# roahmlab/armour

Hardware: AMD Instinct MI355X
Metric: planning iters/s (eval_g+jac) Kinova 7-DOF, 100 timesteps × 20 obstacles (higher is better)
Workload: dtype f64

## Files before the change

### armour_amd/_lib.py

```python
import ctypes as C
import os

_HERE = os.path.dirname(os.path.abspath(__file__))
KEY128 = os.environ.get("ARMOUR_KEY128", "0") not in ("", "0")
LIB_PATH = os.environ.get("ARMOUR_HIP_LIB") or os.path.join(_HERE, "lib", "libarmour_hip_k128.so" if KEY128 else "libarmour_hip.so")

MAXJ = 9
MAXF = 8 if KEY128 else 7

OK, EINVAL, EDEVICE, ECAPACITY, ESTATE = 0, -1, -2, -3, -4
ROADMAP_KNN_MAX = 64
ROADMAP_KNN_MANY = 2048
TREE_NOT_FOUND, TREE_FOUND, TREE_START_BLOCKED, TREE_GOAL_BLOCKED, TREE_FULL = 0, 1, 2, 3, 4
TREE_MAX_NODES, TREE_MAX_ITERATIONS = 8192, 100000
SHORTCUT_OK, SHORTCUT_INVALID = 0, 1
SHORTCUT_MAX_POINTS, SHORTCUT_MAX_PASSES = 1024, 8


class ArmourRobot(C.Structure):
    _fields_ = [
        ("num_joints", C.c_int32), ("num_factors", C.c_int32),
        ("axes", C.c_int32 * MAXJ), ("continuous", C.c_int32 * MAXF),
        ("trans", C.c_double * ((MAXJ + 1) * 3)), ("rots", C.c_double * (MAXJ * 3)),
        ("mass", C.c_double * MAXJ), ("mass_uncertainty", C.c_double),
# ... 75 lines not shown
OPT_P1_TWO_PASS = 106
OPT_P1_STEP_PAIRS = 107
OPT_P1_STEP_QUEUE = 109
OPT_P1_STEP_TAIL_CROSS = 108
OPT_P1_STEP_TWO_CU = 123
OPT_P1_STEP_LEAN_BACK = 124
OPT_P1_TV_TAIL_CROSS = 121
OPT_P1_TV_MIN_GROUPS = 110
OPT_P1_TV_WAVES = 111
OPT_P1_TV_FREE = 112
OPT_P1_TV_SPLIT_FK = 113
OPT_P1_TV_DEDICATED = 114
OPT_P1_TV_HELP_SHIFT = 115
OPT_P1_TV_HELPERS = 116
OPT_P1_TV_HELP_MIN = 117
OPT_P1_TV_HELP_N = 118
OPT_P1_TV_AUX3 = 119
OPT_P1_FULL_PLANES = 120
OPT_P1_TV_ROW_WIDTH = 122
OPT_P2_EX = 130
OPT_STEPS_GRAPH_MIN = 131
OPT_PINNED_MODE = 132
OPT_CULL_ROWS = 133
OPT_SOLVE_SUB_TILES = 140
OPT_SOLVE_DEVICE = 141
OPT_SOLVE_CUT_TILES = 142
OPT_SOLVE_BLOCKS = 143
OPT_SOLVE_SUB_BATCH = 144
OPT_SOLVE_ROW_CAP = 145
OPT_SOLVE_HARD_CAP_S = 146
OPT_SOLVE_WAVES_PER_SIMD = 147
OPT_SOLVE_CULL = 148

EXPORTS = [
    "armour_robot_kinova_gen3_no_gripper", "armour_robot_kinova_gen3_gripper", "armour_robot_fetch", "armour_robot_fetch8", "armour_params_default", "armour_create", "armour_destroy",
    "armour_last_error", "armour_device_available", "armour_alloc_pinned", "armour_free_pinned", "armour_set_problems", "armour_set_problems_armtd", "armour_get_sizes",
    "armour_get_bounds", "armour_eval_f", "armour_eval_grad_f", "armour_eval_g_jac",
    "armour_eval_g_jac_device", "armour_eval_g_jac_device_steps", "armour_prepare_steps", "armour_eval_g_jac_device_multi", "armour_desired_trajectory", "armour_robust_controller", "armour_check_feasible", "armour_get_torque_radius",
    "armour_get_link_generators", "armour_get_link_centers", "armour_get_pz", "armour_get_table_sizes",
    "armour_solve_options_default", "armour_solve", "armour_debug_qp", "armour_debug_qp_box", "armour_debug_qp_elastic", "armour_debug_qp_device", "armour_debug_pz_op",
    "armour_get_hyperplanes", "armour_get_build_ms", "armour_get_build_info", "armour_p2_kernel_name", "armour_debug_load_tables",
    "armour_get_plane_skip", "armour_get_prune_margin", "armour_batch_get_prune_margin", "armour_set_option", "armour_get_option", "armour_controller_set_kernel", "armour_device_memory", "armour_abi_max_factors", "armour_eval_violations_device", "armour_eval_violations", "armour_get_row_relevance", "armour_get_solver_rows",
    "armour_batch_partition", "armour_batch_create", "armour_batch_destroy", "armour_batch_set_option", "armour_batch_set_problems",
    "armour_batch_get_sizes", "armour_batch_get_bounds", "armour_batch_eval_g_jac", "armour_batch_eval_violations", "armour_batch_solve",
    "armour_batch_get_build_ms", "armour_batch_get_build_info",
    "armour_roadmap_create", "armour_roadmap_destroy", "armour_roadmap_get_sizes", "armour_roadmap_check", "armour_roadmap_plan",
# ... 184 lines not shown
```

### armour_amd/csrc/api.hip

```cpp
#include <algorithm>
#include <cmath>
#include <cstdarg>
#include <chrono>
#include <cstring>
#include <mutex>
#include <new>

#include "../../include/armour_robot_fetch.h"
#include "../../include/armour_robot_kinova.h"
#include "bezier.h"
#include "cacc.h"
#include "common.h"
#include "solver_common.h"

static thread_local char g_err[512] = "";

void armour_set_error(const char* fmt, ...) {
    va_list ap;
    va_start(ap, fmt);
    vsnprintf(g_err, sizeof(g_err), fmt, ap);
    va_end(ap);
}

extern "C" const char* armour_last_error(void) { return g_err; }

extern "C" void armour_robot_kinova_gen3_no_gripper(ArmourRobot* robot) { armour_fill_kinova_gen3_no_gripper(robot); }
extern "C" void armour_robot_kinova_gen3_gripper(ArmourRobot* robot) { armour_fill_kinova_gen3_gripper(robot); }
extern "C" void armour_robot_fetch(ArmourRobot* robot) { armour_fill_fetch(robot); }
extern "C" int armour_robot_fetch8(ArmourRobot* robot) {
#if ARMOUR_MAX_FACTORS >= 8
    if (!robot) { armour_set_error("null argument"); return ARMOUR_EINVAL; }
    armour_fill_fetch8(robot);
    return ARMOUR_OK;
#else
    (void)robot;
// ... 78 lines not shown
    tb.row0 = h->row0; tb.mode = h->mode;
    tb.link_count = h->d_link_count; tb.link_center = h->d_link_center; tb.link_indep = h->d_link_indep;
    tb.link_keys = h->d_link_keys; tb.link_coeff = h->d_link_coeff;
    tb.tq_count = h->d_tq_count; tb.tq_center = h->d_tq_center; tb.tq_indep = h->d_tq_indep;
    tb.tq_keys = h->d_tq_keys; tb.tq_coeff = h->d_tq_coeff;
    tb.planes = h->d_planes; tb.planes_ll = h->d_planes_ll; tb.ll_shared = h->ll_shared;
    tb.ex_allowed = h->tune(ARMOUR_OPT_P2_EX);
    tb.obs_center = (h->d_from_center && (h->B >= 8 || !h->planes_have_d)) ? h->d_obs_center : nullptr;
    tb.plane_skip = h->d_plane_skip; tb.bez = h->d_bez;
    for (int i = 0; i < ARMOUR_MAX_FACTORS; i++) tb.k_range[i] = h->params.k_range[i];
    tb.duration = h->params.duration;
    return tb;
}

namespace {
struct TuningSpec { int option; double def, lo, hi; };
const TuningSpec kTuning[] = {
    {ARMOUR_OPT_P1_STEP_WAVES, 0, 0, 4}, {ARMOUR_OPT_P1_STEP_FREE, 1, 0, 1}, {ARMOUR_OPT_P1_STEP_SPLIT_FK, -1, -1, 1}, {ARMOUR_OPT_P1_STEP_AUX3, 1, 0, 1},
    {ARMOUR_OPT_P1_MAX_WAVES_PER_CU, 4, 1, 8}, {ARMOUR_OPT_P1_TWO_PASS, 1, 0, 1}, {ARMOUR_OPT_P1_STEP_PAIRS, 1, 0, 2}, {ARMOUR_OPT_P1_STEP_QUEUE, 1, 0, 3}, {ARMOUR_OPT_P1_STEP_TAIL_CROSS, 0, 0, 514}, {ARMOUR_OPT_P1_STEP_TWO_CU, 3, 0, 33}, {ARMOUR_OPT_P1_STEP_LEAN_BACK, 1, 0, 3}, {ARMOUR_OPT_P1_TV_TAIL_CROSS, 111, 0, 514} ,
    {ARMOUR_OPT_P1_TV_MIN_GROUPS, 31, 1, 1e6}, {ARMOUR_OPT_P1_TV_WAVES, 0, 0, 8}, {ARMOUR_OPT_P1_TV_FREE, 1, 0, 1}, {ARMOUR_OPT_P1_TV_SPLIT_FK, -1, -1, 1},
    {ARMOUR_OPT_P1_TV_DEDICATED, 1, 0, 1}, {ARMOUR_OPT_P1_TV_HELP_SHIFT, 0, 0, 3}, {ARMOUR_OPT_P1_TV_HELPERS, 1, 0, 31}, {ARMOUR_OPT_P1_TV_HELP_MIN, 192, 1, 1e6},
    {ARMOUR_OPT_P1_TV_HELP_N, 1, 0, 1}, {ARMOUR_OPT_P1_TV_AUX3, 1, 0, 1}, {ARMOUR_OPT_P1_TV_ROW_WIDTH, 0, 0, 64}, {ARMOUR_OPT_P1_FULL_PLANES, 0, 0, 1},
    {ARMOUR_OPT_P2_EX, 1, 0, 1}, {ARMOUR_OPT_STEPS_GRAPH_MIN, 2, 0, 1e6}, {ARMOUR_OPT_PINNED_MODE, 0, 0, 2}, {ARMOUR_OPT_CULL_ROWS, 0, 0, 1},
    {ARMOUR_OPT_SOLVE_SUB_TILES, 48, 1, 1e6}, {ARMOUR_OPT_SOLVE_DEVICE, 1, 0, 2}, {ARMOUR_OPT_SOLVE_CUT_TILES, 156, 1, 1e6}, {ARMOUR_OPT_SOLVE_BLOCKS, 0, 0, 1e6},
    {ARMOUR_OPT_SOLVE_SUB_BATCH, 0, 0, 1e6}, {ARMOUR_OPT_SOLVE_ROW_CAP, 0, 0, 1e7}, {ARMOUR_OPT_SOLVE_HARD_CAP_S, 0, 0, 1e6}, {ARMOUR_OPT_SOLVE_WAVES_PER_SIMD, 0, 0, 2}, {ARMOUR_OPT_SOLVE_CULL, -1, -1, 1},
};
const TuningSpec* tuning_spec(int option) {
    for (const TuningSpec& t : kTuning) if (t.option == option) return &t;
    return nullptr;
}
}
void armour_tuning_defaults(double* tuning) {
    for (int o = ARMOUR_OPT_FIRST_TUNING; o <= ARMOUR_OPT_LAST_TUNING; o++) tuning[o - ARMOUR_OPT_FIRST_TUNING] = 0.0;
    for (const TuningSpec& t : kTuning) tuning[t.option - ARMOUR_OPT_FIRST_TUNING] = t.def;
}
bool armour_trace_p1() { static const bool on = getenv("ARMOUR_P1_TRACE") != nullptr; return on; }
BuildStamps& armour_build_stamps() { static thread_local BuildStamps s; return s; }
void armour_build_stamp(const char* name) {
    if (!armour_trace_p1()) return;
    BuildStamps& s = armour_build_stamps();
    if (s.n < 12) { s.t[s.n] = std::chrono::duration<double, std::micro>(std::chrono::steady_clock::now().time_since_epoch()).count(); s.name[s.n] = name; s.n++; }
}
static void armour_build_stamps_print(const char* what) {
    if (!armour_trace_p1()) return;
    BuildStamps& s = armour_build_stamps();
    fprintf(stderr, "[%s, host side, us]", what);
// ... 51 lines not shown
    return ARMOUR_OK;
}

double* armour_handle_pinned(ArmourPlanner* h, int slot, size_t bytes) {
    if (h->solve_pin[slot] && h->solve_pin_bytes[slot] >= bytes) return static_cast<double*>(h->solve_pin[slot]);
    if (h->solve_pin[slot]) { armour_free_pinned(h->solve_pin[slot]); h->solve_pin[slot] = nullptr; h->solve_pin_bytes[slot] = 0; }
    void* p = nullptr;
    if (armour_alloc_pinned(bytes, &p) != ARMOUR_OK) return nullptr;
    h->solve_pin[slot] = p; h->solve_pin_bytes[slot] = bytes;
    return static_cast<double*>(p);
}

static void drop_step_graphs(ArmourPlanner* h) {
    for (auto& g : h->step_graphs) (void)hipGraphExecDestroy(g.exec);
    h->step_graphs.clear();
}

extern "C" void armour_destroy(ArmourPlanner* h) {
    if (!h) return;
    (void)hipSetDevice(h->device);
    if (h->stream) (void)hipStreamSynchronize(h->stream);
    drop_step_graphs(h);
    for (void* pin : h->solve_pin) armour_free_pinned(pin);
    armour_p1_free(h);
    if (h->stream) (void)hipStreamDestroy(h->stream);
    delete h;
}

static int begin_problem_set(ArmourPlanner* h, int B, int O, const double* q0, const double* qd0, const double* qdd0,
                             const double* q_des, int mode = ARMOUR_MODE_ARMOUR) {
    if (!h || !q0 || !qd0 || !qdd0 || !q_des) { armour_set_error("null argument"); return ARMOUR_EINVAL; }
    if (B < 1 || O < 0) { armour_set_error("bad batch/obstacle count (B=%d, O=%d)", B, O); return ARMOUR_EINVAL; }
    {
        const double* arrs[4] = {q0, qd0, qdd0, q_des};
        const size_t bn = (size_t)B * h->n;
        for (int a = 0; a < 4; a++)
            if (const size_t i = first_nonfinite(arrs[a], bn); i < bn) { armour_set_error("non-finite entry in the initial state / goal arrays (array %d, entry %zu)", a, i); return ARMOUR_EINVAL; }
    }
    HIPCHK(hipSetDevice(h->device));
    h->ready = false;
    h->rel.fresh = false; h->rel2.fresh = false;
    h->bounds_on_device = false; h->bounds_on_host = false;
    h->tables_from_host = false;
    h->stats_fresh = false;
    drop_step_graphs(h);
    int rc = ensure_capacity(h, B, O);
// ... 336 lines not shown
            }
    return enqueue_steps(h, d_k, steps, d_g, d_jac, st);
}

extern "C" int armour_eval_g_jac_device_multi(ArmourPlanner* h, const double* d_k, int32_t points, double* d_g, double* d_jac,
                                              void* stream) {
    NEED_READY(h);
    if (!d_k || points < 0) { armour_set_error("bad argument"); return ARMOUR_EINVAL; }
    if (points == 0) return ARMOUR_OK;
    const P2Tables tb = armour_make_tables(h);
    const long long bn = (long long)h->B * h->n, bm = (long long)h->B * h->m;
    return armour_p2_launch(tb, h->max_link, h->max_torque, h->h_plane_skip.data(), d_k, d_g, d_jac, stream ? (hipStream_t)stream : h->stream,
                            points, bn, bm, bm * h->n);
}

int armour_spin_on_stream(hipStream_t st) {
    for (;;) {
        const hipError_t q = hipStreamQuery(st);
        if (q == hipSuccess) return ARMOUR_OK;
        if (q != hipErrorNotReady) { armour_set_error("hipStreamQuery failed: %s", hipGetErrorString(q)); return ARMOUR_EDEVICE; }
    }
}

extern "C" int armour_eval_g_jac(ArmourPlanner* h, const double* k, double* g, double* jac) {
    NEED_READY(h);
    if (!k) { armour_set_error("k is null"); return ARMOUR_EINVAL; }
    HIPCHK(hipSetDevice(h->device));
    const size_t bn = (size_t)h->B * h->n, bm = (size_t)h->B * h->m;
    const P2Tables tb = armour_make_tables(h);
    const int pinned_mode = h->tune(ARMOUR_OPT_PINNED_MODE);
    const bool all_pinned = in_pinned(k, bn * sizeof(double)) && in_pinned(g, bm * sizeof(double)) && in_pinned(jac, bm * h->n * sizeof(double));
    if (all_pinned && pinned_mode == 1) {
        int rc = armour_p2_launch(tb, h->max_link, h->max_torque, h->h_plane_skip.data(), k, g, jac, h->stream);
        if (rc != ARMOUR_OK) return rc;
        return armour_spin_on_stream(h->stream);
    }
    const double* k_dev = h->d_k;
    if (all_pinned && pinned_mode == 2) k_dev = k;
    else HIPCHK(hipMemcpyAsync(h->d_k, k, bn * sizeof(double), hipMemcpyHostToDevice, h->stream));
    int rc = armour_p2_launch(tb, h->max_link, h->max_torque, h->h_plane_skip.data(), k_dev, g ? h->d_g : nullptr, jac ? h->d_jac : nullptr, h->stream);
    if (rc != ARMOUR_OK) return rc;
    if (g && jac && jac == g + bm) {
        HIPCHK(hipMemcpyAsync(g, h->d_g, bm * (1 + (size_t)h->n) * sizeof(double), hipMemcpyDeviceToHost, h->stream));
        return armour_spin_on_stream(h->stream);
    }
    if (g) HIPCHK(hipMemcpyAsync(g, h->d_g, bm * sizeof(double), hipMemcpyDeviceToHost, h->stream));
    if (jac) HIPCHK(hipMemcpyAsync(jac, h->d_jac, bm * h->n * sizeof(double), hipMemcpyDeviceToHost, h->stream));
    return armour_spin_on_stream(h->stream);
}

extern "C" int armour_check_feasible(ArmourPlanner* h, const double* g, int32_t* feasible) {
    NEED_READY(h);
    const slv::RowRule R = armour_row_rule(h);
    const slv::RowLimits L = armour_row_limits(h);
    for (int b = 0; b < h->B; b++) {
        const double* gb = g + (size_t)b * R.m;
        const double* tr = torque_radius_of(h, b);
        bool ok = true;
        for (int r = 0; r < R.m && ok; r++) {
            double l, u;
            slv::row_bounds(R, L, r, tr, &l, &u);
            ok = !slv::outside_slack(R, r, gb[r], l, u);
        }
        feasible[b] = ok ? 1 : 0;
// ... 90 lines not shown
    armour_set_error("armour_get_option: unknown option %d", option);
    return ARMOUR_EINVAL;
}

namespace {
struct ViolArgs {
    slv::RowRule rule;
    const double* g; const double* lo; const double* hi;
    ArmourViolation* out;
};
__global__ __launch_bounds__(256) void armour_violation_kernel(ViolArgs a) {
    __shared__ slv::ViolShared<1> sh;
    const int b = blockIdx.x, tid = threadIdx.x, m = a.rule.m;
    const double* g = a.g + (size_t)b * m;
    const double* lo = a.lo + (size_t)b * m;
    const double* hi = a.hi + (size_t)b * m;
    slv::ViolPartial p[1];
    for (int r = tid; r < m; r += 256) p[0].take(a.rule, r, g[r], lo[r], hi[r]);
    slv::ViolPartial::tree_reduce(sh, p, tid);
    if (tid == 0) a.out[b] = slv::ViolPartial::finish(sh, 0);
}
}

static int eval_violations_device_impl(ArmourPlanner* h, const double* d_k, ArmourViolation* d_out, void* stream, bool allow_cull) {
    NEED_READY(h);
    if (!d_k || !d_out) { armour_set_error("null argument"); return ARMOUR_EINVAL; }
    HIPCHK(hipSetDevice(h->device));
    int rc = armour_upload_bounds(h);
    if (rc != ARMOUR_OK) return rc;
    const hipStream_t st = stream ? (hipStream_t)stream : h->stream;
    if (allow_cull && h->tune(ARMOUR_OPT_CULL_ROWS)) return armour_eval_violations_culled(h, d_k, d_out, st);
    const P2Tables tb = armour_make_tables(h);
    rc = armour_p2_launch(tb, h->max_link, h->max_torque, h->h_plane_skip.data(), d_k, h->d_g, nullptr, st);
    if (rc != ARMOUR_OK) return rc;
    ViolArgs a;
    a.rule = armour_row_rule(h);
    a.g = h->d_g; a.lo = h->d_bounds; a.hi = h->d_bounds + (size_t)h->B * h->m; a.out = d_out;
    hipLaunchKernelGGL(armour_violation_kernel, dim3(h->B), dim3(256), 0, st, a);
    HIPCHK(hipGetLastError());
    return ARMOUR_OK;
}

extern "C" int armour_eval_violations_device(ArmourPlanner* h, const double* d_k, ArmourViolation* d_out, void* stream) {
    return eval_violations_device_impl(h, d_k, d_out, stream, true);
}

extern "C" int armour_eval_violations(ArmourPlanner* h, const double* k, ArmourViolation* out) {
    NEED_READY(h);
    if (!k || !out) { armour_set_error("null argument"); return ARMOUR_EINVAL; }
    HIPCHK(hipSetDevice(h->device));
    const size_t bn = (size_t)h->B * h->n;
    ARMOUR_TRY(h->d_viol.reserve((size_t)h->B));
    double* hk = armour_handle_pinned(h, 6, bn * sizeof(double));
    ArmourViolation* hv = reinterpret_cast<ArmourViolation*>(armour_handle_pinned(h, 7, (size_t)h->B * sizeof(ArmourViolation)));
    if (!hk || !hv) return ARMOUR_EDEVICE;
    memcpy(hk, k, bn * sizeof(double));
    HIPCHK(hipMemcpyAsync(h->d_k, hk, bn * sizeof(double), hipMemcpyHostToDevice, h->stream));
    bool in_box = true;
    for (size_t i = 0; i < bn && in_box; i++) in_box = fabs(k[i]) <= 1.0;
    int rc = eval_violations_device_impl(h, h->d_k, h->d_viol, h->stream, in_box);
    if (rc != ARMOUR_OK) return rc;
    HIPCHK(hipMemcpyAsync(hv, h->d_viol, (size_t)h->B * sizeof(ArmourViolation), hipMemcpyDeviceToHost, h->stream));
    rc = armour_spin_on_stream(h->stream);
    if (rc != ARMOUR_OK) return rc;
    memcpy(out, hv, (size_t)h->B * sizeof(ArmourViolation));
    return ARMOUR_OK;
}

extern "C" int armour_get_torque_radius(ArmourPlanner* h, double* out) {
    NEED_READY(h);
    memcpy(out, h->h_torque_radius.data(), h->h_torque_radius.size() * sizeof(double));
    return ARMOUR_OK;
}

extern "C" int armour_get_link_generators(ArmourPlanner* h, double* out) {
    NEED_READY(h);
    memcpy(out, h->h_link_gens.data(), h->h_link_gens.size() * sizeof(double));
    return ARMOUR_OK;
}

extern "C" int armour_get_link_centers(ArmourPlanner* h, const double* k, double* centers) {
    NEED_READY(h);
    HIPCHK(hipSetDevice(h->device));
// ... 120 lines not shown
```

### armour_amd/csrc/common.h

```cpp
#pragma once

#include <hip/hip_runtime.h>

#include <cstdint>
#include <cstdio>
#include <string>
#include <vector>

#include "../../include/armour_hip.h"
#include "device_mem.h"
#include "row_rules.h"

#define ARMOUR_NPLANES 36
#define ARMOUR_PLANE_COMPONENTS 5

#define ARMOUR_FIRST_LL_PLANE 21
#define ARMOUR_N_LL_PLANES 15
__host__ __device__ inline int armour_row_stride(int Q) { return (Q + 15) & ~15; }
__host__ __device__ inline size_t armour_planes_ab_offset(int Q) { (void)Q; return 0; }
__host__ __device__ inline size_t armour_planes_cd_offset(int Q) { return (size_t)2 * ARMOUR_NPLANES * armour_row_stride(Q); }
__host__ __device__ inline size_t armour_planes_dll_offset(int Q) { return (size_t)4 * ARMOUR_NPLANES * armour_row_stride(Q); }
__host__ __device__ inline size_t armour_planes_d_offset(int Q) { return (size_t)(4 * ARMOUR_NPLANES + 16) * armour_row_stride(Q); }
__host__ __device__ inline size_t armour_planes_per_problem(int Q) { return (size_t)(5 * ARMOUR_NPLANES + 16) * armour_row_stride(Q); }
__host__ __device__ inline size_t armour_plane_index(int Q, int q, int p, int c) {
// ... 56 lines not shown
    DevBuf<int> extra;
    std::vector<int> h_count, h_tq_count;
    int max_count = 0;
    bool fresh = false;
    double ms = 0;
};

struct ArmourPlanner {
    ArmourRobot robot;
    ArmourParams params;
    ArmourLimits lim;
    ArmourUltimateBound ub;
    int device = 0;
    hipStream_t stream = nullptr;
    int T = 0, J = 0, n = 0;
    int B = 0, O = 0, Q = 0, m = 0;
    bool ready = false;
    int mode = ARMOUR_MODE_ARMOUR;
    bool no_torque() const { return mode == ARMOUR_MODE_ARMTD || params.input_constraints_off != 0; }
    int continuous_mask() const { int mk = 0; for (int i = 0; i < n; i++) if (robot.continuous[i]) mk |= 1 << i; return mk; }
    int row0 = 0;
    std::vector<double> h_krange;
    DevBuf<double> d_jrs;
    void* solve_pin[10] = {nullptr, nullptr, nullptr, nullptr, nullptr, nullptr, nullptr, nullptr, nullptr, nullptr};
    size_t solve_pin_bytes[10] = {0, 0, 0, 0, 0, 0, 0, 0, 0, 0};
    bool stats_fresh = false;
    int opt_p1_build = 0;
    double opt_p1_work_mb = 0;
    int opt_p1_keep_work = 1;
    double tuning[ARMOUR_OPT_LAST_TUNING - ARMOUR_OPT_FIRST_TUNING + 1];
    int tune(int option) const { return (int)tuning[option - ARMOUR_OPT_FIRST_TUNING]; }
    double tune_f(int option) const { return tuning[option - ARMOUR_OPT_FIRST_TUNING]; }
    DevBuf<ArmourViolation> d_viol;
    RelLists rel, rel2;
    int rel2_tq_cap = 0;
    DevBuf<unsigned char> d_sweep;
    SolveDeviceWork solve_dev;
    DevBuf<double> d_bounds;
    bool bounds_on_device = false, bounds_on_host = false;
    bool tables_from_host = false;
    std::vector<double> h_gl, h_gu;
    std::vector<double> h_q0, h_qd0, h_qdd0, h_qdes;
    std::vector<double> h_torque_radius;
    DevBuf<double> d_tr_stage;
    std::vector<double> h_link_gens;
    std::vector<unsigned long long> h_plane_skip;
    std::vector<double> h_prune_margin;
    int allocB = 0, allocO = 0;
// ... 18 lines not shown
    DevBuf<unsigned long long> d_plane_skip;
    DevBuf<double> d_bez;
    DevBuf<double> d_k;
    DevBuf<double> d_g;
    double* d_jac = nullptr;
    double build_ms = 0;
    int p1_step_cap_hint = 0, p1_tv_shape_hint = 0;
    bool p1_two_cu_off = false;
    int p1_hint_B = 0, p1_hint_T = 0, p1_hint_O = 0, p1_hint_builds = 0;
    int build_info[4] = {0, 0, 0, 0};
    int max_link = 0, max_torque = 0;
    long long sum_link = 0, sum_torque = 0;
    void* p1 = nullptr;
    struct StepsGraph { const double* d_k; int steps; double* d_g; double* d_jac; hipGraphExec_t exec; unsigned long long last_use; };
    std::vector<StepsGraph> step_graphs;
    unsigned long long graph_clock = 0;
};

void armour_tuning_defaults(double* tuning);
bool armour_trace_p1();
bool armour_trace_solve();

int armour_p2_launch(const P2Tables& tb, int max_link, int max_torque, const unsigned long long* h_skip, const double* d_k, double* d_g, double* d_jac, hipStream_t stream,
                     int steps = 1, long long k_stride = 0, long long g_stride = 0, long long j_stride = 0, bool skip_collision_blocks = false);
int armour_relevance_build(ArmourPlanner* h, bool for_solver);
int armour_eval_violations_culled(ArmourPlanner* h, const double* d_k, ArmourViolation* d_out, hipStream_t st);
int armour_refresh_table_stats(ArmourPlanner* h);
int armour_checked_collision_rows(const ArmourPlanner* h);
slv::RowRule armour_row_rule(const ArmourPlanner* h);
slv::RowLimits armour_row_limits(const ArmourPlanner* h);
#define NEED_READY(h)                                                                        \
    if (!(h)) { armour_set_error("null handle"); return ARMOUR_EINVAL; }                     \
    if (!(h)->ready) { armour_set_error("no problem set: call armour_set_problems first"); return ARMOUR_ESTATE; }
void armour_plan_coeffs(const ArmourPlanner* h, size_t ix, double c[3]);
double* armour_handle_pinned(ArmourPlanner* h, int slot, size_t bytes);
int armour_p2_slice_links_launch(const P2Tables& tb, const double* d_k, double* d_centers, hipStream_t stream);
P2Tables armour_make_tables(const ArmourPlanner* h);
int armour_upload_bounds(ArmourPlanner* h);
struct BuildStamps { double t[12]; const char* name[12]; int n; };
BuildStamps& armour_build_stamps();
void armour_build_stamp(const char* name);
int armour_bounds_launch(ArmourPlanner* h, const double* d_torque_radius);

int armour_p1_build(ArmourPlanner* h, const double* obstacles);
void armour_p1_free(ArmourPlanner* h);
int armour_p1_full_planes(ArmourPlanner* h, double* d_full);

// ... 8 lines not shown
```

### armour_amd/csrc/p2_eval.hip

```cpp
#include "p2_tiles.h"

using namespace p2;

namespace {

template <bool WANT_G, bool WANT_J, bool MULTI, bool DFC, bool LL, int PPW, bool EX>
__global__ __launch_bounds__(P2_BLOCK) __attribute__((amdgpu_waves_per_eu(P2_WPE(DFC, MULTI)))) void armour_p2_eval_kernel(P2Tables tb, const double* __restrict__ k_all,
                                                                  double* __restrict__ g_all, double* __restrict__ jac_all,
                                                                  P2Launch lp) {
    extern __shared__ __attribute__((aligned(16))) unsigned char smem_raw[];
    const int b = blockIdx.y, role = blockIdx.x + lp.role0;
    const int n = tb.n, m = tb.m;
    const double* k0 = k_all + (size_t)b * n;
    double* g0 = WANT_G ? g_all + (size_t)b * m : nullptr;
    double* jac0 = WANT_J ? jac_all + (size_t)b * m * n : nullptr;
    const double k_first = ((int)threadIdx.x < n) ? k0[threadIdx.x] : 0.0;
#ifdef P2_ABLATE
    if ((P2_ABLATE & 1) && role < lp.nbc) return;
    if ((P2_ABLATE & 2) && role >= lp.nbc && role < lp.nbc + lp.nbt) return;
    if ((P2_ABLATE & 4) && role >= lp.nbc + lp.nbt) return;
#endif
    if (role < lp.nbc) collision_block<WANT_G, WANT_J, MULTI, DFC, LL, PPW, EX>(tb, lp, b, role, k0, k_first, g0, jac0, smem_raw);
    else if (role < lp.nbc + lp.nbt) torque_block<WANT_G, WANT_J, MULTI, DFC, LL, PPW, EX>(tb, lp, b, role, k0, k_first, g0, jac0, smem_raw);
    else limit_block<WANT_G, WANT_J, MULTI, DFC, LL, PPW, EX>(tb, lp, b, role, k0, k_first, g0, jac0, smem_raw);
}

__global__ void armour_p2_slice_links_kernel(P2Tables tb, const double* __restrict__ k_all, double* __restrict__ centers) {
    __shared__ KPow kp;
    const int b = blockIdx.y;
    fill_kpow(kp, threadIdx.x < (unsigned)tb.n ? k_all[(size_t)b * tb.n + threadIdx.x] : 0.0, tb.n);
    __syncthreads();
    const int task = blockIdx.x * blockDim.x + threadIdx.x;
    const int JT = tb.J * tb.T;
    if (task >= JT * 3) return;
    const int lt = task / 3, e = task - lt * 3;
    const size_t idx = (size_t)b * JT + lt;
    const int cnt = tb.link_count[idx];
    double cen = tb.link_center[idx * 3 + e];
    for (int mo = 0; mo < cnt; mo++)
        cen += mono_value(kp, tb.link_keys[idx * tb.capL + mo], tb.link_coeff[(idx * tb.capL + mo) * 3 + e], tb.n);
    const int l = lt / tb.T, t = lt - l * tb.T;
    centers[(((size_t)b * tb.T + t) * tb.J + l) * 3 + e] = interval_center(cen, tb.link_indep[idx * 3 + e]);
}

}

const char* armour_p2_kernel_name(void) { return "armour_p2_eval_kernel"; }
// ... 24 lines not shown
    lp.skip_by_value = (tb.B == 1 && h_skip) ? 1 : 0;
    lp.skip0 = lp.skip_by_value ? h_skip[0] : 0ull;
    lp.steps = steps; lp.k_stride = k_stride; lp.g_stride = g_stride; lp.j_stride = j_stride;
    lp.magic_O = div_magic(tb.O > 0 ? tb.O : 1); lp.magic_pp3 = div_magic(3 * lp.strideL);
    if (tb.Q >= (1 << 20)) { armour_set_error("more than 2^20 collision rows per problem"); return ARMOUR_ECAPACITY; }
    if (lp.strideL * 3 > P2_BLOCK * P2_TASK_ROUNDS) { armour_set_error("link PZ with %d monomials exceeds the P2 kernel's %d", lp.strideL, P2_BLOCK * P2_TASK_ROUNDS / 3); return ARMOUR_ECAPACITY; }
    lp.pair_chunk = std::max(1, std::min(std::min(lp.max_pairs, P2_BLOCK / P2_SL), (P2_BLOCK * P2_TASK_ROUNDS) / (lp.strideL * 3)));
    if (lp.strideT > 32 * P2_TQ_ROUNDS) { armour_set_error("torque PZ with %d monomials exceeds the P2 kernel's %d", lp.strideT, 32 * P2_TQ_ROUNDS); return ARMOUR_ECAPACITY; }
    const size_t col = ((size_t)lp.max_pairs * P2_SL + (size_t)lp.pair_chunk * lp.strideL * P2_SL + 4 * 64 * 4 + 64 * ARMOUR_MAX_FACTORS) * sizeof(double) + 4 * 64 * sizeof(int);
    const size_t tq = (size_t)P2_TQ_ROWS * lp.strideT * P2_TQW * sizeof(double);
    const size_t lim = (size_t)2 * ARMOUR_MAX_FACTORS * 8 * sizeof(double);
    const size_t smem = 2 * sizeof(KPow) + std::max(std::max(col, tq), lim);
    if (smem > 64 * 1024) { armour_set_error("P2 kernel needs %zu B of LDS (link/torque monomial counts too large)", smem); return ARMOUR_ECAPACITY; }
    const bool dfc = tb.obs_center != nullptr && tb.ll_shared;
    bool six = h_skip != nullptr;
    for (int b = 0; six && b < tb.B; b++) six = __builtin_popcountll(~h_skip[b] & ((1ull << ARMOUR_NPLANES) - 1ull)) <= 24;
    bool exact = six && tb.ex_allowed && lp.max_pairs <= lp.pair_chunk;
    for (int b = 0; exact && b < tb.B; b++) exact = armour_p2_ex_layout_ok(h_skip[b]);
    *lp_out = lp; *smem_out = smem; *dfc_out = dfc; *six_out = six; *exact_out = exact;
    return ARMOUR_OK;
}

int armour_p2_launch(const P2Tables& tb, int max_link, int max_torque, const unsigned long long* h_skip, const double* d_k, double* d_g, double* d_jac,
                     hipStream_t stream, int steps, long long k_stride, long long g_stride, long long j_stride, bool skip_collision_blocks) {
    if (!d_g && !d_jac) return ARMOUR_OK;
    P2Launch lp;
    size_t smem = 0;
    bool dfc, six, exact;
    const int rc = armour_p2_plan(tb, max_link, max_torque, h_skip, steps, k_stride, g_stride, j_stride, &lp, &smem, &dfc, &six, &exact);
    if (rc != ARMOUR_OK) return rc;
    if (skip_collision_blocks) lp.role0 = lp.nbc;
    dim3 grid(lp.nbc + lp.nbt + 1 - lp.role0, tb.B), block(P2_BLOCK);
#define P2_LAUNCH_M(G, J, M)                                                                                                                      \
    do {                                                                                                                                          \
        if (dfc && exact && !(M)) hipLaunchKernelGGL((armour_p2_eval_kernel<G, J, false, true, true, 6, true>), grid, block, smem, stream, tb, d_k, d_g, d_jac, lp);      \
        else if (dfc && six) hipLaunchKernelGGL((armour_p2_eval_kernel<G, J, M, true, true, 6, false>), grid, block, smem, stream, tb, d_k, d_g, d_jac, lp);                \
        else if (dfc) hipLaunchKernelGGL((armour_p2_eval_kernel<G, J, M, true, true, 9, false>), grid, block, smem, stream, tb, d_k, d_g, d_jac, lp);              \
        else if (tb.ll_shared && exact && !(M)) hipLaunchKernelGGL((armour_p2_eval_kernel<G, J, false, false, true, 6, true>), grid, block, smem, stream, tb, d_k, d_g, d_jac, lp); \
        else if (tb.ll_shared && six) hipLaunchKernelGGL((armour_p2_eval_kernel<G, J, M, false, true, 6, false>), grid, block, smem, stream, tb, d_k, d_g, d_jac, lp); \
        else if (tb.ll_shared) hipLaunchKernelGGL((armour_p2_eval_kernel<G, J, M, false, true, 9, false>), grid, block, smem, stream, tb, d_k, d_g, d_jac, lp); \
        else hipLaunchKernelGGL((armour_p2_eval_kernel<G, J, M, false, false, 9, false>), grid, block, smem, stream, tb, d_k, d_g, d_jac, lp);             \
    } while (0)
#define P2_LAUNCH(G, J)                                                                                                     \
    do {                                                                                                                    \
        if (steps > 1) P2_LAUNCH_M(G, J, true); else P2_LAUNCH_M(G, J, false);                                                                         \
    } while (0)
    if (d_g && d_jac) P2_LAUNCH(true, true);
    else if (d_g) P2_LAUNCH(true, false);
    else P2_LAUNCH(false, true);
#undef P2_LAUNCH
#undef P2_LAUNCH_M
    HIPCHK(hipGetLastError());
    return ARMOUR_OK;
}

// ... 8 lines not shown
```

### include/armour_hip.h

```cpp
#ifndef ARMOUR_HIP_H
#define ARMOUR_HIP_H

#include <stdint.h>
#include "armour_types.h"

#ifdef __cplusplus
extern "C" {
#endif

#define ARMOUR_OK 0
#define ARMOUR_EINVAL (-1)
#define ARMOUR_EDEVICE (-2)
#define ARMOUR_ECAPACITY (-3)
#define ARMOUR_ESTATE (-4)

typedef struct ArmourPlanner ArmourPlanner;

typedef struct ArmourLimits {
    int32_t max_batch;
    int32_t max_obstacles;
    int32_t link_monomials;
    int32_t torque_monomials;
    int32_t work_monomials;
    int32_t raw_terms;
// ... 26 lines not shown
#define ARMOUR_OPT_P1_TWO_PASS 106
#define ARMOUR_OPT_P1_STEP_TAIL_CROSS 108
#define ARMOUR_OPT_P1_STEP_QUEUE 109
#define ARMOUR_OPT_P1_STEP_PAIRS 107
#define ARMOUR_OPT_P1_STEP_TWO_CU 123
#define ARMOUR_OPT_P1_STEP_LEAN_BACK 124
#define ARMOUR_OPT_P1_TV_MIN_GROUPS 110
#define ARMOUR_OPT_P1_TV_WAVES 111
#define ARMOUR_OPT_P1_TV_FREE 112
#define ARMOUR_OPT_P1_TV_SPLIT_FK 113
#define ARMOUR_OPT_P1_TV_DEDICATED 114
#define ARMOUR_OPT_P1_TV_HELP_SHIFT 115
#define ARMOUR_OPT_P1_TV_HELPERS 116
#define ARMOUR_OPT_P1_TV_HELP_MIN 117
#define ARMOUR_OPT_P1_TV_HELP_N 118
#define ARMOUR_OPT_P1_TV_AUX3 119
#define ARMOUR_OPT_P1_TV_TAIL_CROSS 121
#define ARMOUR_OPT_P1_TV_ROW_WIDTH 122
#define ARMOUR_OPT_P1_FULL_PLANES 120
#define ARMOUR_OPT_P2_EX 130
#define ARMOUR_OPT_STEPS_GRAPH_MIN 131
#define ARMOUR_OPT_CULL_ROWS 133
#define ARMOUR_OPT_PINNED_MODE 132
#define ARMOUR_OPT_SOLVE_SUB_TILES 140
#define ARMOUR_OPT_SOLVE_DEVICE 141
#define ARMOUR_OPT_SOLVE_CUT_TILES 142
#define ARMOUR_OPT_SOLVE_BLOCKS 143
#define ARMOUR_OPT_SOLVE_SUB_BATCH 144
#define ARMOUR_OPT_SOLVE_ROW_CAP 145
#define ARMOUR_OPT_SOLVE_HARD_CAP_S 146
#define ARMOUR_OPT_SOLVE_WAVES_PER_SIMD 147
#define ARMOUR_OPT_SOLVE_CULL 148
#define ARMOUR_OPT_FIRST_TUNING 101
#define ARMOUR_OPT_LAST_TUNING 148
int armour_device_memory(int32_t device, uint64_t* free_bytes, uint64_t* total_bytes);
int armour_abi_max_factors(void);
int armour_set_option(ArmourPlanner* h, int32_t option, double value);
int armour_get_option(ArmourPlanner* h, int32_t option, double* value);

int armour_set_problems(ArmourPlanner* h, int32_t B, int32_t O, const double* q0, const double* qd0,
                        const double* qdd0, const double* q_des, const double* obstacles);

int armour_set_problems_armtd(ArmourPlanner* h, int32_t B, int32_t O, const double* q0, const double* qd0, const double* q_des,
                              const double* jrs, const double* k_range, const double* obstacles);

int armour_get_sizes(const ArmourPlanner* h, int32_t* B, int32_t* n, int32_t* m);
// ... 238 lines not shown
```

Before: 161,500.

## Pass k as kernel argument and stage device-to-host readback through pinned buffer

For single-problem evaluation, the trajectory parameters k are packed into a by-value kernel argument struct, which removes the separate host-to-device copy before the P2 evaluation kernel. The g/jacobian readback now goes through a pinned staging buffer, optionally in chunks with events, and each chunk is scattered into the caller's pageable buffers with memcpy. This targets the latency of pageable transfers and an extra copy per call on a small workload. It adds a new kernel variant, an extra host memcpy, and busy-polling on events.

```diff
diff --git a/armour_amd/_lib.py b/armour_amd/_lib.py
--- a/armour_amd/_lib.py
+++ b/armour_amd/_lib.py
@@ -121,6 +121,8 @@
 OPT_STEPS_GRAPH_MIN = 131
 OPT_PINNED_MODE = 132
 OPT_CULL_ROWS = 133
+OPT_HOST_K_INLINE = 134
+OPT_HOST_COPY_CHUNKS = 135
 OPT_SOLVE_SUB_TILES = 140
 OPT_SOLVE_DEVICE = 141
 OPT_SOLVE_CUT_TILES = 142
diff --git a/armour_amd/csrc/api.hip b/armour_amd/csrc/api.hip
--- a/armour_amd/csrc/api.hip
+++ b/armour_amd/csrc/api.hip
@@ -11,6 +11,7 @@
 #include "bezier.h"
 #include "cacc.h"
 #include "common.h"
+#include "host_stage.h"
 #include "solver_common.h"
 
 static thread_local char g_err[512] = "";
@@ -135,6 +136,7 @@
     {ARMOUR_OPT_P1_TV_DEDICATED, 1, 0, 1}, {ARMOUR_OPT_P1_TV_HELP_SHIFT, 0, 0, 3}, {ARMOUR_OPT_P1_TV_HELPERS, 1, 0, 31}, {ARMOUR_OPT_P1_TV_HELP_MIN, 192, 1, 1e6},
     {ARMOUR_OPT_P1_TV_HELP_N, 1, 0, 1}, {ARMOUR_OPT_P1_TV_AUX3, 1, 0, 1}, {ARMOUR_OPT_P1_TV_ROW_WIDTH, 0, 0, 64}, {ARMOUR_OPT_P1_FULL_PLANES, 0, 0, 1},
     {ARMOUR_OPT_P2_EX, 1, 0, 1}, {ARMOUR_OPT_STEPS_GRAPH_MIN, 2, 0, 1e6}, {ARMOUR_OPT_PINNED_MODE, 0, 0, 2}, {ARMOUR_OPT_CULL_ROWS, 0, 0, 1},
+    {ARMOUR_OPT_HOST_K_INLINE, 1, 0, 1}, {ARMOUR_OPT_HOST_COPY_CHUNKS, 1, 0, 64},
     {ARMOUR_OPT_SOLVE_SUB_TILES, 48, 1, 1e6}, {ARMOUR_OPT_SOLVE_DEVICE, 1, 0, 2}, {ARMOUR_OPT_SOLVE_CUT_TILES, 156, 1, 1e6}, {ARMOUR_OPT_SOLVE_BLOCKS, 0, 0, 1e6},
     {ARMOUR_OPT_SOLVE_SUB_BATCH, 0, 0, 1e6}, {ARMOUR_OPT_SOLVE_ROW_CAP, 0, 0, 1e7}, {ARMOUR_OPT_SOLVE_HARD_CAP_S, 0, 0, 1e6}, {ARMOUR_OPT_SOLVE_WAVES_PER_SIMD, 0, 0, 2}, {ARMOUR_OPT_SOLVE_CULL, -1, -1, 1},
 };
@@ -232,6 +234,7 @@
     if (h->stream) (void)hipStreamSynchronize(h->stream);
     drop_step_graphs(h);
     for (void* pin : h->solve_pin) armour_free_pinned(pin);
+    for (hipEvent_t e : h->stage_events) (void)hipEventDestroy(e);
     armour_p1_free(h);
     if (h->stream) (void)hipStreamDestroy(h->stream);
     delete h;
@@ -614,6 +617,41 @@
     }
 }
 
+static int staged_read_back(ArmourPlanner* h, double* g, double* jac, size_t g_bytes, size_t jac_bytes, int chunks) {
+    const hstage::Plan pl = hstage::plan(g_bytes, jac_bytes, g != nullptr, jac != nullptr, chunks);
+    unsigned char* stage = reinterpret_cast<unsigned char*>(armour_handle_pinned(h, 10, g_bytes + jac_bytes));
+    if (!stage) return ARMOUR_EDEVICE;
+    while ((int)h->stage_events.size() + 1 < pl.count) {
+        hipEvent_t e = nullptr;
+        HIPCHK(hipEventCreateWithFlags(&e, hipEventDisableTiming));
+        h->stage_events.push_back(e);
+    }
+    const unsigned char* dev = reinterpret_cast<const unsigned char*>(h->d_g.p);
+    for (int i = 0; i < pl.count; i++) {
+        size_t b, e;
+        hstage::chunk_range(pl, i, &b, &e);
+        HIPCHK(hipMemcpyAsync(stage + b, dev + b, e - b, hipMemcpyDeviceToHost, h->stream));
+        if (i + 1 < pl.count) HIPCHK(hipEventRecord(h->stage_events[i], h->stream));
+    }
+    for (int i = 0; i + 1 < pl.count; i++) {
+        for (;;) {
+            const hipError_t q = hipEventQuery(h->stage_events[i]);
+            if (q == hipSuccess) break;
+            if (q != hipErrorNotReady) { armour_set_error("hipEventQuery failed: %s", hipGetErrorString(q)); return ARMOUR_EDEVICE; }
+        }
+        size_t b, e;
+        hstage::chunk_range(pl, i, &b, &e);
+        hstage::scatter(stage, b, e, g_bytes, g, jac);
+    }
+    ARMOUR_TRY(armour_spin_on_stream(h->stream));
+    if (pl.count) {
+        size_t b, e;
+        hstage::chunk_range(pl, pl.count - 1, &b, &e);
+        hstage::scatter(stage, b, e, g_bytes, g, jac);
+    }
+    return ARMOUR_OK;
+}
+
 extern "C" int armour_eval_g_jac(ArmourPlanner* h, const double* k, double* g, double* jac) {
     NEED_READY(h);
     if (!k) { armour_set_error("k is null"); return ARMOUR_EINVAL; }
@@ -628,10 +666,18 @@
         return armour_spin_on_stream(h->stream);
     }
     const double* k_dev = h->d_k;
+    const double* k_inline = nullptr;
     if (all_pinned && pinned_mode == 2) k_dev = k;
+    else if (h->B == 1 && h->tune(ARMOUR_OPT_HOST_K_INLINE)) k_inline = k;
     else HIPCHK(hipMemcpyAsync(h->d_k, k, bn * sizeof(double), hipMemcpyHostToDevice, h->stream));
-    int rc = armour_p2_launch(tb, h->max_link, h->max_torque, h->h_plane_skip.data(), k_dev, g ? h->d_g : nullptr, jac ? h->d_jac : nullptr, h->stream);
-    if (rc != ARMOUR_OK) return rc;
+    int rc = armour_p2_launch(tb, h->max_link, h->max_torque, h->h_plane_skip.data(), k_dev, g ? h->d_g : nullptr, jac ? h->d_jac : nullptr, h->stream,
+                              1, 0, 0, 0, false, k_inline);
+    if (rc != ARMOUR_OK) return rc;
+    const int chunks = h->tune(ARMOUR_OPT_HOST_COPY_CHUNKS);
+    const size_t g_bytes = bm * sizeof(double), jac_bytes = bm * h->n * sizeof(double);
+    if (chunks > 0 && g_bytes + jac_bytes <= hstage::kMaxBytes && h->d_jac == h->d_g + bm &&
+        !(in_pinned(g, g_bytes) && in_pinned(jac, jac_bytes)))
+        return staged_read_back(h, g, jac, g_bytes, jac_bytes, chunks);
     if (g && jac && jac == g + bm) {
         HIPCHK(hipMemcpyAsync(g, h->d_g, bm * (1 + (size_t)h->n) * sizeof(double), hipMemcpyDeviceToHost, h->stream));
         return armour_spin_on_stream(h->stream);
@@ -768,7 +814,7 @@
 }
 }
 
-static int eval_violations_device_impl(ArmourPlanner* h, const double* d_k, ArmourViolation* d_out, void* stream, bool allow_cull) {
+static int eval_violations_device_impl(ArmourPlanner* h, const double* d_k, ArmourViolation* d_out, void* stream, bool allow_cull, const double* k_host = nullptr) {
     NEED_READY(h);
     if (!d_k || !d_out) { armour_set_error("null argument"); return ARMOUR_EINVAL; }
     HIPCHK(hipSetDevice(h->device));
@@ -777,7 +823,7 @@
     const hipStream_t st = stream ? (hipStream_t)stream : h->stream;
     if (allow_cull && h->tune(ARMOUR_OPT_CULL_ROWS)) return armour_eval_violations_culled(h, d_k, d_out, st);
     const P2Tables tb = armour_make_tables(h);
-    rc = armour_p2_launch(tb, h->max_link, h->max_torque, h->h_plane_skip.data(), d_k, h->d_g, nullptr, st);
+    rc = armour_p2_launch(tb, h->max_link, h->max_torque, h->h_plane_skip.data(), d_k, h->d_g, nullptr, st, 1, 0, 0, 0, false, k_host);
     if (rc != ARMOUR_OK) return rc;
     ViolArgs a;
     a.rule = armour_row_rule(h);
@@ -800,11 +846,14 @@
     double* hk = armour_handle_pinned(h, 6, bn * sizeof(double));
     ArmourViolation* hv = reinterpret_cast<ArmourViolation*>(armour_handle_pinned(h, 7, (size_t)h->B * sizeof(ArmourViolation)));
     if (!hk || !hv) return ARMOUR_EDEVICE;
-    memcpy(hk, k, bn * sizeof(double));
-    HIPCHK(hipMemcpyAsync(h->d_k, hk, bn * sizeof(double), hipMemcpyHostToDevice, h->stream));
     bool in_box = true;
     for (size_t i = 0; i < bn && in_box; i++) in_box = fabs(k[i]) <= 1.0;
-    int rc = eval_violations_device_impl(h, h->d_k, h->d_viol, h->stream, in_box);
+    const bool k_inline = h->B == 1 && h->tune(ARMOUR_OPT_HOST_K_INLINE) && !(in_box && h->tune(ARMOUR_OPT_CULL_ROWS));
+    if (!k_inline) {
+        memcpy(hk, k, bn * sizeof(double));
+        HIPCHK(hipMemcpyAsync(h->d_k, hk, bn * sizeof(double), hipMemcpyHostToDevice, h->stream));
+    }
+    int rc = eval_violations_device_impl(h, h->d_k, h->d_viol, h->stream, in_box, k_inline ? k : nullptr);
     if (rc != ARMOUR_OK) return rc;
     HIPCHK(hipMemcpyAsync(hv, h->d_viol, (size_t)h->B * sizeof(ArmourViolation), hipMemcpyDeviceToHost, h->stream));
     rc = armour_spin_on_stream(h->stream);
diff --git a/armour_amd/csrc/common.h b/armour_amd/csrc/common.h
--- a/armour_amd/csrc/common.h
+++ b/armour_amd/csrc/common.h
@@ -102,8 +102,9 @@
     int row0 = 0;
     std::vector<double> h_krange;
     DevBuf<double> d_jrs;
-    void* solve_pin[10] = {nullptr, nullptr, nullptr, nullptr, nullptr, nullptr, nullptr, nullptr, nullptr, nullptr};
-    size_t solve_pin_bytes[10] = {0, 0, 0, 0, 0, 0, 0, 0, 0, 0};
+    void* solve_pin[11] = {nullptr, nullptr, nullptr, nullptr, nullptr, nullptr, nullptr, nullptr, nullptr, nullptr, nullptr};
+    size_t solve_pin_bytes[11] = {0, 0, 0, 0, 0, 0, 0, 0, 0, 0, 0};
+    std::vector<hipEvent_t> stage_events;
     bool stats_fresh = false;
     int opt_p1_build = 0;
     double opt_p1_work_mb = 0;
@@ -168,7 +169,8 @@
 bool armour_trace_solve();
 
 int armour_p2_launch(const P2Tables& tb, int max_link, int max_torque, const unsigned long long* h_skip, const double* d_k, double* d_g, double* d_jac, hipStream_t stream,
-                     int steps = 1, long long k_stride = 0, long long g_stride = 0, long long j_stride = 0, bool skip_collision_blocks = false);
+                     int steps = 1, long long k_stride = 0, long long g_stride = 0, long long j_stride = 0, bool skip_collision_blocks = false,
+                     const double* k_host = nullptr);
 int armour_relevance_build(ArmourPlanner* h, bool for_solver);
 int armour_eval_violations_culled(ArmourPlanner* h, const double* d_k, ArmourViolation* d_out, hipStream_t st);
 int armour_refresh_table_stats(ArmourPlanner* h);
diff --git a/armour_amd/csrc/host_stage.h b/armour_amd/csrc/host_stage.h
--- /dev/null
+++ b/armour_amd/csrc/host_stage.h
@@ -0,0 +1,44 @@
+#pragma once
+#include <cstddef>
+#include <cstring>
+
+namespace hstage {
+
+constexpr size_t kMaxBytes = (size_t)4 << 20;
+constexpr size_t kAlign = 256;
+
+struct Plan {
+    size_t lo = 0, hi = 0;
+    size_t chunk = 0;
+    int count = 0;
+};
+
+inline Plan plan(size_t g_bytes, size_t jac_bytes, bool want_g, bool want_jac, int chunks) {
+    Plan p;
+    p.lo = want_g ? 0 : g_bytes;
+    p.hi = want_jac ? g_bytes + jac_bytes : g_bytes;
+    if (p.hi <= p.lo) { p.hi = p.lo; return p; }
+    const size_t len = p.hi - p.lo, c = chunks > 1 ? (size_t)chunks : 1;
+    p.chunk = ((len + c - 1) / c + kAlign - 1) / kAlign * kAlign;
+    p.count = (int)((len + p.chunk - 1) / p.chunk);
+    return p;
+}
+
+inline void chunk_range(const Plan& p, int i, size_t* begin, size_t* end) {
+    const size_t b = p.lo + (size_t)i * p.chunk, e = b + p.chunk;
+    *begin = b < p.hi ? b : p.hi;
+    *end = e < p.hi ? e : p.hi;
+}
+
+inline void scatter(const unsigned char* stage, size_t begin, size_t end, size_t g_bytes, void* g, void* jac) {
+    if (begin < g_bytes && g) {
+        const size_t e = end < g_bytes ? end : g_bytes;
+        if (e > begin) memcpy(static_cast<unsigned char*>(g) + begin, stage + begin, e - begin);
+    }
+    if (end > g_bytes && jac) {
+        const size_t b = begin > g_bytes ? begin : g_bytes;
+        if (end > b) memcpy(static_cast<unsigned char*>(jac) + (b - g_bytes), stage + b, end - b);
+    }
+}
+
+}
diff --git a/armour_amd/csrc/p2_eval.hip b/armour_amd/csrc/p2_eval.hip
--- a/armour_amd/csrc/p2_eval.hip
+++ b/armour_amd/csrc/p2_eval.hip
@@ -23,6 +23,30 @@
     if (role < lp.nbc) collision_block<WANT_G, WANT_J, MULTI, DFC, LL, PPW, EX>(tb, lp, b, role, k0, k_first, g0, jac0, smem_raw);
     else if (role < lp.nbc + lp.nbt) torque_block<WANT_G, WANT_J, MULTI, DFC, LL, PPW, EX>(tb, lp, b, role, k0, k_first, g0, jac0, smem_raw);
     else limit_block<WANT_G, WANT_J, MULTI, DFC, LL, PPW, EX>(tb, lp, b, role, k0, k_first, g0, jac0, smem_raw);
+}
+
+struct P2KInline { double k[ARMOUR_MAX_FACTORS]; };
+
+template <bool WANT_G, bool WANT_J, bool DFC, bool LL, int PPW, bool EX>
+__global__ __launch_bounds__(P2_BLOCK) __attribute__((amdgpu_waves_per_eu(P2_WPE(DFC, false)))) void armour_p2_eval_kv_kernel(P2Tables tb, const double* __restrict__ k_all,
+                                                                  double* __restrict__ g_all, double* __restrict__ jac_all,
+                                                                  P2Launch lp, P2KInline kin) {
+    extern __shared__ __attribute__((aligned(16))) unsigned char smem_raw[];
+    (void)k_all;
+    const int role = blockIdx.x + lp.role0;
+    double* g0 = WANT_G ? g_all : nullptr;
+    double* jac0 = WANT_J ? jac_all : nullptr;
+    double k_first = 0.0;
+#pragma unroll
+    for (int j = 0; j < ARMOUR_MAX_FACTORS; j++) k_first = ((int)threadIdx.x == j) ? kin.k[j] : k_first;
+    if (role < lp.nbc) collision_block<WANT_G, WANT_J, false, DFC, LL, PPW, EX>(tb, lp, 0, role, nullptr, k_first, g0, jac0, smem_raw);
+    else if (role < lp.nbc + lp.nbt) torque_block<WANT_G, WANT_J, false, DFC, LL, PPW, EX>(tb, lp, 0, role, nullptr, k_first, g0, jac0, smem_raw);
+    else {
+        double* k_lds = reinterpret_cast<double*>(smem_raw);
+        if ((int)threadIdx.x < ARMOUR_MAX_FACTORS) k_lds[threadIdx.x] = k_first;
+        __syncthreads();
+        limit_block<WANT_G, WANT_J, false, DFC, LL, PPW, EX>(tb, lp, 0, role, k_lds, k_first, g0, jac0, smem_raw);
+    }
 }
 
 __global__ void armour_p2_slice_links_kernel(P2Tables tb, const double* __restrict__ k_all, double* __restrict__ centers) {
@@ -93,7 +117,7 @@
 }
 
 int armour_p2_launch(const P2Tables& tb, int max_link, int max_torque, const unsigned long long* h_skip, const double* d_k, double* d_g, double* d_jac,
-                     hipStream_t stream, int steps, long long k_stride, long long g_stride, long long j_stride, bool skip_collision_blocks) {
+                     hipStream_t stream, int steps, long long k_stride, long long g_stride, long long j_stride, bool skip_collision_blocks, const double* k_host) {
     if (!d_g && !d_jac) return ARMOUR_OK;
     P2Launch lp;
     size_t smem = 0;
@@ -102,6 +126,31 @@
     if (rc != ARMOUR_OK) return rc;
     if (skip_collision_blocks) lp.role0 = lp.nbc;
     dim3 grid(lp.nbc + lp.nbt + 1 - lp.role0, tb.B), block(P2_BLOCK);
+    if (k_host && tb.B == 1 && steps == 1) {
+        if (!d_g && !dfc && !six) HIPCHK(hipMemcpyAsync(const_cast<double*>(d_k), k_host, (size_t)tb.n * sizeof(double), hipMemcpyHostToDevice, stream));
+        else {
+            P2KInline kin;
+            for (int j = 0; j < ARMOUR_MAX_FACTORS; j++) kin.k[j] = j < tb.n ? k_host[j] : 0.0;
+#define P2_LAUNCH_KV(G, J)                                                                                                                        \
+    do {                                                                                                                                          \
+        if (dfc && exact) hipLaunchKernelGGL((armour_p2_eval_kv_kernel<G, J, true, true, 6, true>), grid, block, smem, stream, tb, d_k, d_g, d_jac, lp, kin);            \
+        else if (dfc && six) hipLaunchKernelGGL((armour_p2_eval_kv_kernel<G, J, true, true, 6, false>), grid, block, smem, stream, tb, d_k, d_g, d_jac, lp, kin);        \
+        else if (dfc) hipLaunchKernelGGL((armour_p2_eval_kv_kernel<G, J, true, true, 9, false>), grid, block, smem, stream, tb, d_k, d_g, d_jac, lp, kin);               \
+        else if (tb.ll_shared && exact) hipLaunchKernelGGL((armour_p2_eval_kv_kernel<G, J, false, true, 6, true>), grid, block, smem, stream, tb, d_k, d_g, d_jac, lp, kin); \
+        else if (tb.ll_shared && six) hipLaunchKernelGGL((armour_p2_eval_kv_kernel<G, J, false, true, 6, false>), grid, block, smem, stream, tb, d_k, d_g, d_jac, lp, kin); \
+        else if constexpr (G) {                                                                                                                   \
+            if (tb.ll_shared) hipLaunchKernelGGL((armour_p2_eval_kv_kernel<G, J, false, true, 9, false>), grid, block, smem, stream, tb, d_k, d_g, d_jac, lp, kin);     \
+            else hipLaunchKernelGGL((armour_p2_eval_kv_kernel<G, J, false, false, 9, false>), grid, block, smem, stream, tb, d_k, d_g, d_jac, lp, kin);                 \
+        }                                                                                                                                         \
+    } while (0)
+            if (d_g && d_jac) P2_LAUNCH_KV(true, true);
+            else if (d_g) P2_LAUNCH_KV(true, false);
+            else P2_LAUNCH_KV(false, true);
+#undef P2_LAUNCH_KV
+            HIPCHK(hipGetLastError());
+            return ARMOUR_OK;
+        }
+    }
 #define P2_LAUNCH_M(G, J, M)                                                                                                                      \
     do {                                                                                                                                          \
         if (dfc && exact && !(M)) hipLaunchKernelGGL((armour_p2_eval_kernel<G, J, false, true, true, 6, true>), grid, block, smem, stream, tb, d_k, d_g, d_jac, lp);      \
diff --git a/include/armour_hip.h b/include/armour_hip.h
--- a/include/armour_hip.h
+++ b/include/armour_hip.h
@@ -72,6 +72,8 @@
 #define ARMOUR_OPT_STEPS_GRAPH_MIN 131
 #define ARMOUR_OPT_CULL_ROWS 133
 #define ARMOUR_OPT_PINNED_MODE 132
+#define ARMOUR_OPT_HOST_K_INLINE 134
+#define ARMOUR_OPT_HOST_COPY_CHUNKS 135
 #define ARMOUR_OPT_SOLVE_SUB_TILES 140
 #define ARMOUR_OPT_SOLVE_DEVICE 141
 #define ARMOUR_OPT_SOLVE_CUT_TILES 142
```

Result: no change. 161,100, median of 2 (-0.2%).
